# HaploConduct/HaploConduct

Measured on AMD Instinct MI355X. Metric: candidate overlaps scored/sec (edge-calc scoring pass: compute_overlap + overlap_score + admission class, candidates resident in HBM; the whole stage from the overlaps text: stage_end_to_end), higher is better.
Workload: dtype f64

## Files before the change

### haploconduct_amd/_native.py

```python
import ctypes as C
import os

_HERE = os.path.dirname(os.path.abspath(__file__))
lib_path = os.path.join(_HERE, "csrc", "libhcedge.so")


class HcError(RuntimeError):
    def __init__(self, status, where=""):
        self.status = status
        try:
            msg = lib.hc_strerror(status).decode()
            detail = lib.hc_last_error().decode()
        except Exception:
            msg, detail = "?", ""
        super().__init__(f"{where}: {msg} ({status}) {detail}".strip())


if not os.path.exists(lib_path):
    raise ImportError(
        f"{lib_path} is missing: build it with `python -c 'import __graft_entry__ as g; g.build()'` "
        "or `make -C haploconduct_amd/csrc`.  haploconduct_amd has no CPU fallback."
    )

try:
# ... 64 lines not shown
    "hc_block_destroy": (C.c_int, [_vp]),
    "hc_text_set_ids": (C.c_int, [_vp, _vp, C.c_uint32]),
    "hc_textblock_create": (C.c_int, [_vp, C.c_uint64, C.POINTER(_vp)]),
    "hc_textblock_buffer": (_vp, [_vp]),
    "hc_textblock_submit": (C.c_int, [_vp, C.c_uint64, C.c_uint64, C.c_uint64]),
    "hc_textblock_submit_from": (C.c_int, [_vp, _vp, C.c_uint64, _vp, C.c_uint64, _vp, C.c_uint64]),
    "hc_linechain_create": (C.c_int, [_vp, C.c_uint64, C.POINTER(_vp)]),
    "hc_linechain_destroy": (C.c_int, [_vp]),
    "hc_textblock_wait": (C.c_int, [_vp, C.POINTER(hc_text_result)]),
    "hc_textblock_list_nonplain": (C.c_int, [_vp, C.c_uint32]),
    "hc_textblock_destroy": (C.c_int, [_vp]),
    "hc_textblock_regrown": (C.c_uint64, [_vp]),
    "hc_textblock_reserve_rows": (C.c_int, [_vp, C.c_uint64]),
    "hc_graph_begin": (C.c_int, [_vp]),
    "hc_graph_append": (C.c_int, [_vp, _vp, C.c_uint64]),
    "hc_graph_resolve": (C.c_int, [_vp, _vp, C.c_uint64, C.c_uint64, _vp, C.c_uint32, C.POINTER(hc_graph_counts)]),
    "hc_graph_fetch": (C.c_int, [_vp, _vp, _vp, _vp, _vp, _vp, _vp, _vp]),
    "hc_reset": (C.c_int, [_vp, _vp]),
    "hc_set_comm_reserve": (C.c_int, [_vp, C.c_uint32]),
    "hc_comm_gate_device": (C.c_int, [_vp, _vp, C.c_uint32]),
    "hc_compact_pack_device": (C.c_int, [_vp, _vp, C.c_uint64, _vp, _vp, C.c_uint64, C.c_uint64, _vp, _vp]),
    "hc_pack_rows_device": (C.c_int, [_vp, _vp, _vp, _vp, C.c_uint64, C.c_uint64, _vp, _vp]),
    "hc_score_batch_compact": (C.c_int, [_vp, _vp, C.c_uint64, _vp, _vp, C.c_uint64, C.POINTER(C.c_uint64)]),
    "hc_set_reorder": (C.c_int, [_vp, C.c_int]),
    "hc_host_alloc": (C.c_int, [_vp, C.POINTER(_vp), C.c_uint64]),
    "hc_host_free": (C.c_int, [_vp, _vp]),
    "hc_time_score_kernel": (C.c_int, [_vp, C.c_uint32, _vp, C.c_uint64, _vp, C.c_int, C.POINTER(C.c_float)]),
    "hc_count_positions_device": (C.c_int, [_vp, C.c_uint32, _vp, C.c_uint64, C.POINTER(C.c_uint64), C.POINTER(C.c_uint64)]),
    "hc_finalize": (C.c_int, [C.POINTER(hc_settings), _vp, C.POINTER(C.c_double), C.POINTER(C.c_double), C.POINTER(C.c_uint32)]),
    "hc_finalize_batch": (C.c_int, [C.POINTER(hc_settings), _vp, C.c_uint64, _vp, _vp, _vp]),
    "hc_get_info": (C.c_int, [_vp, C.POINTER(C.c_uint32), C.POINTER(C.c_uint64)] + [C.POINTER(C.c_double)] * 4),
    "hc_get_kernel_info": (C.c_int, [_vp, C.c_char_p, C.c_uint32]),
    "hc_get_kernel_info_for": (C.c_int, [_vp, C.c_uint64, C.c_char_p, C.c_uint32]),
    "hc_dev_radix_sort": (C.c_int, [C.c_uint32, C.c_uint32, _vp, _vp, _vp, _vp, C.c_uint64, C.c_int, C.c_int]),
    "hc_dev_exclusive_sum": (C.c_int, [C.c_uint32, _vp, _vp, C.c_uint64]),
    "hc_dev_select_flagged": (C.c_int, [_vp, C.c_uint64, _vp, C.POINTER(C.c_uint64)]),
    "hc_dev_unique_u64": (C.c_int, [_vp, C.c_uint64, _vp, C.POINTER(C.c_uint64)]),
}
for _name, (_res, _args) in _sig.items():
    _f = getattr(lib, _name)
    _f.restype = _res
    _f.argtypes = _args


def check(status, where=""):
    if status != 0:
        raise HcError(status, where)


def device_count():
    return int(lib.hc_device_count())


def version():
    return lib.hc_version().decode()
```

### haploconduct_amd/csrc/hc_api.cpp

```cpp
#include <hip/hip_runtime.h>

#include <chrono>
#include <cmath>
#include <cstdio>
#include <cstdlib>
#include <cstring>
#include <thread>
#include <array>
#include <limits>
#include <new>
#include <string>
#include <vector>

#include "../../include/hcedge.h"
#include "hc_ctx.h"

static thread_local std::string g_last_error;

static int fail(int status, const std::string& what) {
    g_last_error = what;
    return status;
}
namespace hc {
int set_last_error(int status, const std::string& what) { return fail(status, what); }
// ... 35 lines not shown
        case HC_ERR_ARG: return "invalid argument";
        case HC_ERR_NOMEM: return "out of memory";
        case HC_ERR_HIP: return "HIP runtime error";
        case HC_ERR_NO_DEVICE: return "no HIP device (libhcedge has no CPU fallback)";
        case HC_ERR_STATE: return "call order violated";
        case HC_ERR_BAD_READ: return "malformed read set";
        case HC_ERR_BAD_OVERLAP: return "malformed overlap record";
        case HC_ERR_IO: return "I/O error";
        case HC_ERR_FORMAT: return "input format the reference rejects";
        case HC_ERR_DATA: return "overlap touches a base/quality the reference asserts on";
        case HC_ERR_NOT_ON_DEVICE: return "not decided on the device (the host's route takes the input)";
        default: return "unknown status";
    }
}

const char* hc_last_error(void) { return g_last_error.c_str(); }

int hc_device_count(void) {
    int n = 0;
    if (hipGetDeviceCount(&n) != hipSuccess) return 0;
    return n;
}

static void apply_settings(hc_ctx* c, const hc_settings* settings) {
    c->settings = *settings;
    c->params.edge = make_band(settings->edge_threshold);
    c->params.ov = make_band(settings->ov_threshold);
    c->params.merge_contigs = settings->merge_contigs;
    c->params.min_read_len = settings->min_read_len;
    c->params.flags = (settings->edge_threshold < 0 ? kParamEdgeAlways : 0u) | (settings->ov_threshold < 0 ? kParamOvAlways : 0u);
    c->params.rec_fmt = HC_REC_FULL;
    c->params.pad = 0;
    c->params.n_dev = nullptr;
}

static int create_ctx(hc_ctx* c, const hc_settings* settings) {
    c->settings = *settings;
    c->device = settings->device;
    HC_HIP(hipSetDevice(c->device));
    hipDeviceProp_t prop;
    HC_HIP(hipGetDeviceProperties(&prop, c->device));
    c->n_cu = prop.multiProcessorCount > 0 ? (uint32_t)prop.multiProcessorCount : 256u;
    HC_HIP(hipStreamCreateWithFlags(&c->stream, hipStreamNonBlocking));
    HC_HIP(hipEventCreate(&c->ev0));
    HC_HIP(hipEventCreate(&c->ev1));
    HC_HIP(hipMalloc((void**)&c->d_totals, 2 * sizeof(unsigned long long)));
    HC_HIP(hc::set_score_kernel_lds_limit());
    apply_settings(c, settings);
    return HC_OK;
}

int hc_create(hc_ctx** out, const hc_settings* settings) {
    if (!out || !settings) return fail(HC_ERR_ARG, "hc_create: null argument");
    *out = nullptr;
    int n = 0;
    if (hipGetDeviceCount(&n) != hipSuccess || n <= 0)
        return fail(HC_ERR_NO_DEVICE, "hc_create: no HIP device visible");
    if (settings->device < 0 || settings->device >= n) return fail(HC_ERR_ARG, "hc_create: device ordinal out of range");
    hc_ctx* c = new (std::nothrow) hc_ctx();
    if (!c) return fail(HC_ERR_NOMEM, "hc_create: host allocation failed");
    const int rc = create_ctx(c, settings);
    if (rc != HC_OK) {
        const std::string why = g_last_error;
        hc_destroy(c);
        return fail(rc, why);
    }
// ... 2 lines not shown
}

static void free_store(hc_ctx* c, bool scratch_too = true) {
    if (scratch_too) {
        for (auto& sl : c->finder_scratch) {
            if (sl.p) (void)hipFree(sl.p);
            sl.p = nullptr;
            sl.cap = 0;
        }
        for (auto& sl : c->ingest_scratch) {
            if (sl.p) (void)hipFree(sl.p);
            sl.p = nullptr;
            sl.cap = 0;
        }
        if (c->d_found_lines) (void)hipFree(c->d_found_lines);
        c->d_found_lines = nullptr;
        c->found_lines_cap = 0;
        if (c->d_found) (void)hipFree(c->d_found);
        c->d_found = nullptr;
        c->found_cap = 0;
    }
    c->n_found = 0;
    c->found_valid = false;
    if (c->d_sym) (void)hipFree(c->d_sym);
    if (c->d_reads) (void)hipFree(c->d_reads);
    if (c->d_lut) (void)hipFree(c->d_lut);
    if (c->d_inv_n) (void)hipFree(c->d_inv_n);
    c->d_inv_n = nullptr;
    c->d_sym = nullptr;
    c->d_reads = nullptr;
    c->d_lut = nullptr;
    c->have_reads = false;
    c->store_bytes = 0;
}

int hc_destroy(hc_ctx* c) {
    if (!c) return HC_OK;
    (void)hipSetDevice(c->device);
    if (c->stream) (void)hipStreamSynchronize(c->stream);
    free_store(c);
    if (c->d_in) (void)hipFree(c->d_in);
    if (c->d_out) (void)hipFree(c->d_out);
    if (c->d_totals) (void)hipFree(c->d_totals);
    if (c->d_started) (void)hipFree(c->d_started);
    if (c->d_sort) (void)hipFree(c->d_sort);
    if (c->d_sort_tmp) (void)hipFree(c->d_sort_tmp);
    if (c->d_compact_tmp) (void)hipFree(c->d_compact_tmp);
    if (c->d_compact_idx) (void)hipFree(c->d_compact_idx);
    if (c->d_compact_res) (void)hipFree(c->d_compact_res);
    if (c->ev0) (void)hipEventDestroy(c->ev0);
    if (c->ev1) (void)hipEventDestroy(c->ev1);
    if (c->scratch_done) (void)hipEventDestroy(c->scratch_done);
    for (int t = 0; t < 2; t++) {
        if (c->graph.h_stage[t]) (void)hipHostFree(c->graph.h_stage[t]);
        if (c->h_ingest[t]) (void)hipHostFree(c->h_ingest[t]);
        if (c->graph.stage_free[t]) (void)hipEventDestroy(c->graph.stage_free[t]);
    }
    for (void* h : c->h_sfo_text)
        if (h) (void)hipHostFree(h);
    for (hipStream_t s : c->text_copy_stream)
        if (s) (void)hipStreamDestroy(s);
    if (c->stream) (void)hipStreamDestroy(c->stream);
    delete c;
    return HC_OK;
}

// ... 232 lines not shown
        for (uint32_t r = 0; r < n_reads; r++) {
            const uint32_t q = read_first_seq[r];
            if (read_first_seq[r + 1] - q == 2) {
                c->seq_refs[q] = hc::SeqRef{sym_off[q], seq_len[q], n_single + pair_no, rc_delta[q], 0};
                c->seq_refs[q + 1] = hc::SeqRef{sym_off[q + 1], seq_len[q + 1], n_single + n_pairs + pair_no, rc_delta[q + 1], 0};
                pair_no++;
            } else {
                c->seq_refs[q] = hc::SeqRef{sym_off[q], seq_len[q], r, rc_delta[q], 0};
            }
        }
    }
    c->view.sym = c->d_sym;
    c->view.reads = c->d_reads;
    c->view.n_reads = n_reads;
    c->view.n_seq = n_seq;
    c->view.K = K;
    c->view.symbytes = symbytes;
    c->view.lut_bytes = (uint32_t)(lut.size() * sizeof(double));
    c->view.inv_n = c->d_inv_n;
    c->view.inv_len = (uint32_t)inv_n.size();
    c->store_bytes = sym_bytes_total;
    c->view.store_bytes = sym_bytes_total;
    {
        bool same_len = n_seq > 0;
        for (uint32_t q = 1; q < n_seq && same_len; q++) same_len = seq_len[q] == seq_len[0];
        uint32_t n_single = 0;
        for (uint32_t r = 0; r < n_reads; r++) n_single += read_first_seq[r + 1] - read_first_seq[r] == 1;
        c->view.regular = (same_len && c->singles_first && !any_bad_base) ? 1u : 0u;
        if (const char* v = getenv("HC_REGULAR_STORE")) c->view.regular = c->view.regular && atoi(v) != 0;
        c->view.ulen = same_len ? seq_len[0] : 0u;
        c->view.n_single = n_single;
        c->view.seq_syms = same_len ? (uint32_t)(2 * hc::slot_stride(seq_len[0], symbytes, slot_align)) : 0u;
    }
    c->have_reads = true;
    {
        uint32_t lmin = 0, lmax = 0;
        if (n_seq) {
            std::vector<uint32_t> sorted_len(seq_len.begin(), seq_len.begin() + n_seq);
            const size_t k5 = (size_t)n_seq * 5 / 100, k95 = std::min<size_t>(n_seq - 1, (size_t)n_seq * 95 / 100);
            std::nth_element(sorted_len.begin(), sorted_len.begin() + k5, sorted_len.end());
            lmin = sorted_len[k5];
            std::nth_element(sorted_len.begin(), sorted_len.begin() + k95, sorted_len.end());
            lmax = sorted_len[k95];
        }
        c->len_p5 = lmin;
        c->len_p95 = lmax;
        c->view.balance = (n_seq && lmax > 2u * lmin && total / n_seq > 350) ? 1u : 0u;
        if (const char* b = getenv("HC_BALANCE")) c->view.balance = atoi(b) != 0;
    }
    c->coop_fetch = true;
    if (const char* v = getenv("HC_FETCH_GROUP")) {
        c->coop_fetch = !strcmp(v, "coop");
        c->fetch_group = atoi(v) == 2 ? 2 : 4;
    } else {
        const uint64_t mean_len = n_seq ? total / n_seq : 0;
        c->fetch_group = (mean_len > 600 || symbytes == 2) ? 2 : 4;
        const uint32_t lmin = c->len_p5, lmax = c->len_p95;
        uint32_t n_pairs = 0;
        for (uint32_t r = 0; r < n_reads; r++) n_pairs += read_first_seq[r + 1] - read_first_seq[r] == 2;
        const bool short_mixed_singles = n_seq && n_pairs == 0 && lmax > 2u * lmin && mean_len <= 300 && !c->view.balance;
        c->coop_fetch = !short_mixed_singles;
        if (short_mixed_singles) c->fetch_group = 2;
    }
    c->view.long_rows = (n_seq && total / n_seq > 600) ? 1u : 0u;
    return HC_OK;
}

static bool host_batch_is_ordered(const void* in, size_t rec_bytes, uint64_t n) {
    if (n < 2) return true;
    const uint64_t samples = n - 1 < 4096 ? n - 1 : 4096;
    const uint64_t step = (n - 2) / samples > 0 ? (n - 2) / samples : 1;
    uint64_t share = 0;
    for (uint64_t k = 0; k < samples; k++) {
        const uint32_t* a = (const uint32_t*)((const char*)in + k * step * rec_bytes);
        const uint32_t* b = (const uint32_t*)((const char*)in + (k * step + 1) * rec_bytes);
        share += (a[0] == b[0]) | (a[0] == b[1]) | (a[1] == b[0]) | (a[1] == b[1]);
    }
    return share * 2 >= samples;
}

static int ensure_sort_workspace(hc_ctx* c, uint64_t n) {
    if (n <= c->sort_cap) return HC_OK;
    if (c->d_sort) (void)hipFree(c->d_sort);
    if (c->d_sort_tmp) (void)hipFree(c->d_sort_tmp);
    c->d_sort = nullptr;
    c->d_sort_tmp = nullptr;
    c->sort_cap = 0;
    c->sort_tmp_bytes = hc::reorder_temp_bytes((uint32_t)n);
    HC_HIP(hipMalloc((void**)&c->d_sort, 4 * n * sizeof(uint32_t)));
    HC_HIP(hipMalloc(&c->d_sort_tmp, c->sort_tmp_bytes ? c->sort_tmp_bytes : 16));
    c->sort_cap = n;
    return HC_OK;
}

}

int hc_ctx_score(hc_ctx* c, uint32_t fmt, const void* d_in, uint64_t n, void* d_out, hipStream_t s, bool reorder,
                 hc_gather_row* rows, unsigned long long* row_count, uint64_t cap, uint64_t base_index, const unsigned long long* n_dev,
                 const hc_line_rec* lines_in, hc_line_rec* lines_out, hc_bucket_ws* bucket) {
    const bool want_perm = reorder && n > 1 && n < (1ull << 31);
    const bool want_bucket = c->view.balance && c->coop_fetch && n < (1ull << 32);
    const bool want_segments = rows && !lines_in && c->coop_fetch;
    const bool ctx_scratch = want_perm || (want_bucket && !bucket) || want_segments;
    if (ctx_scratch) {
        if (!c->scratch_done) HC_HIP(hipEventCreateWithFlags(&c->scratch_done, hipEventDisableTiming));
        if (c->scratch_used && c->scratch_stream != s) HC_HIP(hipStreamWaitEvent(s, c->scratch_done, 0));
    }
    const uint32_t* perm = nullptr;
    if (want_perm) {
        int rc = ensure_sort_workspace(c, n);
        if (rc) return rc;
        uint32_t* keys_in = c->d_sort;
        uint32_t* keys_out = c->d_sort + c->sort_cap;
        uint32_t* idx_in = c->d_sort + 2 * c->sort_cap;
        uint32_t* perm_out = c->d_sort + 3 * c->sort_cap;
        HC_HIP(hc::launch_reorder(c->view.n_reads, fmt, d_in, (uint32_t)n, keys_in, keys_out, idx_in, perm_out, c->d_sort_tmp,
                                  c->sort_tmp_bytes, s));
        perm = perm_out;
    }
    hc::ScoreParams prm = c->params;
    prm.rec_fmt = fmt;
    prm.pad = 0;
    prm.n_dev = n_dev;
    uint32_t *bperm = nullptr, *bqueue = nullptr;
    if (want_bucket) {
        hc_bucket_ws* ws = bucket ? bucket : &c->bucket;
        int rc = ws->ensure(n);
        if (rc) return rc;
        bperm = ws->perm();
        bqueue = ws->queue();
    }
    hc_gather_row* seg_buf = nullptr;
    uint32_t* seg_count = nullptr;
    uint64_t seg_total = 0;
    if (want_segments) {
        seg_total = 2 * cap + hc::kSinkMaxGroups * 512;
        if (seg_total * sizeof(hc_gather_row) > c->sink_rows.cap && c->scratch_used) HC_HIP(hipEventSynchronize(c->scratch_done));
        int rc = c->sink_rows.ensure(seg_total * sizeof(hc_gather_row));
        if (rc) return rc;
        if (!c->sink_counts.p) {
            if ((rc = c->sink_counts.ensure((hc::kSinkMaxGroups + 2) * sizeof(uint32_t))) != HC_OK) return rc;
            HC_HIP(hipMemsetAsync(c->sink_counts.p, 0, (hc::kSinkMaxGroups + 2) * sizeof(uint32_t), s));
        }
        seg_buf = c->sink_rows.as<hc_gather_row>();
        seg_count = c->sink_counts.as<uint32_t>();
    }
    if (want_segments && c->sink_dirty) {
        HC_HIP(hipMemsetAsync(c->sink_counts.as<uint32_t>() + hc::kSinkMaxGroups, 0, 2 * sizeof(uint32_t), s));
        c->sink_dirty = false;
    }
    const uint32_t cus = c->comm_reserve && c->comm_reserve < c->n_cu ? c->n_cu - c->comm_reserve : c->n_cu;
    unsigned long long* started = (rows && !lines_in) ? c->d_started : nullptr;
    uint32_t started_groups = 0;
    const hipError_t le = hc::launch_score(c->view, prm, c->d_lut, d_in, n, (hc_result_rec*)d_out, perm, cus, c->coop_fetch ? 0 : c->fetch_group, c->fetch_group, rows,
                                           row_count, cap, base_index, s, lines_in, lines_out, bperm, bqueue, seg_buf, seg_count, seg_total, &c->sink_turn, started,
                                           &started_groups);
    if (le != hipSuccess) {
        if (want_segments) c->sink_dirty = true;
        return hc::set_last_error(HC_ERR_HIP, std::string("launch_score: ") + hipGetErrorString(le));
    }
    if (started) c->started_target += started_groups;
    if (ctx_scratch) {
        HC_HIP(hipEventRecord(c->scratch_done, s));
        c->scratch_stream = s;
        c->scratch_used = true;
    }
    return HC_OK;
}

extern "C" {

int hc_set_reorder(hc_ctx* c, int mode) {
    if (!c || mode < HC_REORDER_NEVER || mode > HC_REORDER_AUTO) return fail(HC_ERR_ARG, "hc_set_reorder: bad argument");
    c->reorder_mode = mode;
    return HC_OK;
}

int hc_score_batch_device(hc_ctx* c, const void* d_in, uint64_t n, void* d_out, void* hip_stream) {
    if (!c) return fail(HC_ERR_ARG, "hc_score_batch_device: null context");
    if (!c->have_reads) return fail(HC_ERR_STATE, "hc_score_batch_device: hc_set_reads has not been called");
    if (n == 0) return HC_OK;
    if (!d_in || !d_out) return fail(HC_ERR_ARG, "hc_score_batch_device: null buffer");
    HC_HIP(hipSetDevice(c->device));
    hipStream_t s = hip_stream ? (hipStream_t)hip_stream : c->stream;
    return hc_ctx_score(c, HC_REC_FULL, d_in, n, d_out, s, c->reorder_mode == HC_REORDER_ALWAYS, nullptr, nullptr, 0, 0);
}

int hc_score_cands_device(hc_ctx* c, const void* d_in, uint64_t n, void* d_out, void* hip_stream) {
    if (!c) return fail(HC_ERR_ARG, "hc_score_cands_device: null context");
    if (!c->have_reads) return fail(HC_ERR_STATE, "hc_score_cands_device: hc_set_reads has not been called");
    if (n == 0) return HC_OK;
    if (!d_in || !d_out) return fail(HC_ERR_ARG, "hc_score_cands_device: null buffer");
    HC_HIP(hipSetDevice(c->device));
    hipStream_t s = hip_stream ? (hipStream_t)hip_stream : c->stream;
    return hc_ctx_score(c, HC_REC_COMPACT, d_in, n, d_out, s, c->reorder_mode == HC_REORDER_ALWAYS, nullptr, nullptr, 0, 0);
}

void hc_pack_cands(const hc_overlap_rec* in, uint64_t n, hc_cand_rec* out) {
    for (uint64_t i = 0; i < n; i++) {
        const hc_overlap_rec& r = in[i];
        const uint32_t p1 = r.pos1 < HC_CAND_POS_MASK ? r.pos1 : HC_CAND_POS_MASK;
        const uint32_t p2 = r.pos2 < HC_CAND_POS_MASK ? r.pos2 : HC_CAND_POS_MASK;
        const uint32_t oc = r.ord == '-' ? 0u : (r.ord == '1' ? 1u : (r.ord == '2' ? 2u : 3u));
        out[i].read1 = r.read1;
        out[i].read2 = r.read2;
        out[i].pos1_bits = p1 | (r.ori1 ? 1u << 28 : 0u) | (r.ori2 ? 1u << 29 : 0u) | (oc << 30);
        out[i].pos2_bits = p2;
// ... 329 lines not shown
```

### haploconduct_amd/csrc/hc_ctx.h

```cpp
#pragma once
#include <hip/hip_runtime.h>

#include <atomic>
#include <string>
#include <vector>

#include "../../include/hcedge.h"
#include "hc_device.h"
#include "hc_overlap_finder.h"

namespace hc {
hipError_t launch_encode(uint32_t symbytes, const uint8_t* bases, const uint8_t* quals, const uint64_t* raw_off,
                         const uint64_t* seq_off, const uint32_t* rc_delta, const uint8_t* qmap, uint32_t n_seq, uint32_t K, void* sym,
                         uint8_t* seq_bad, const uint32_t* read_first_seq, uint32_t n_reads, ReadDesc* descs, uint32_t slot_align,
                         hipStream_t stream);
hipError_t launch_score(const StoreView& st, const ScoreParams& prm, const double* lut_g, const void* in, uint64_t n,
                        hc_result_rec* out, const uint32_t* perm, uint32_t n_cu, int fetch_group, int lane_fetch_group, hc_gather_row* rows,
                        unsigned long long* row_count, uint64_t cap, uint64_t base_index, hipStream_t stream,
                        const hc_line_rec* lines_in = nullptr, hc_line_rec* lines_out = nullptr, uint32_t* bucket_perm = nullptr,
                        uint32_t* bucket_queue = nullptr, hc_gather_row* seg_buf = nullptr, uint32_t* seg_count = nullptr, uint64_t seg_total_rows = 0,
                        uint32_t* spill_turn = nullptr, unsigned long long* started = nullptr, uint32_t* started_groups = nullptr);
hipError_t set_score_kernel_lds_limit();
std::string describe_score_kernel(const StoreView& st, int fetch_group, int lane_fetch_group, uint32_t n_cu = 256, uint64_t n = 0);
size_t compact_temp_bytes(uint32_t n);
hipError_t launch_compact(const hc_result_rec* res, uint32_t n, uint32_t* idx_out, unsigned long long* count_out, void* temp,
                          size_t temp_bytes, hipStream_t stream);
hipError_t launch_narrow_payload(const void* in32, uint64_t cap, void* out24, uint32_t n_cu, hipStream_t stream);
hipError_t launch_pack_rows(const hc_result_rec* res, const uint32_t* idx, const unsigned long long* count, uint64_t cap, uint64_t base,
                            hc_gather_row* rows, uint32_t n_cu, hipStream_t stream);
hipError_t launch_pack_header(const unsigned long long* count, hc_gather_row* header, hipStream_t stream);
hipError_t launch_gather_results(const hc_result_rec* res, const uint32_t* idx, const unsigned long long* count,
                                 hc_result_rec* out, uint32_t n_cu, hipStream_t stream);
size_t reorder_temp_bytes(uint32_t n);
hipError_t launch_reorder(uint32_t n_reads, uint32_t fmt, const void* in, uint32_t n, uint32_t* keys_in, uint32_t* keys_out,
                          uint32_t* idx_in, uint32_t* perm_out, void* temp, size_t temp_bytes, hipStream_t stream);
hipError_t launch_count_positions(const StoreView& st, uint32_t min_read_len, uint32_t fmt, const void* in, uint64_t n,
                                  unsigned long long* totals, hipStream_t stream);
hipError_t launch_kept_rows(const hc_result_rec* res, uint64_t n, const unsigned long long* n_dev, uint64_t base_index, uint32_t* tile_cnt,
                            uint32_t* tile_off, hc_gather_row* rows, uint64_t cap, unsigned long long* count, const hc_line_rec* lines_in,
                            hc_line_rec* lines_out, hipStream_t stream, const uint32_t* text_tally = nullptr,
                            unsigned long long* text_counters = nullptr);
hipError_t launch_flush_text_rows(const void* rows, void* rows_mapped, const void* lines, void* lines_mapped, const unsigned long long* count,
                                  uint64_t cap, const unsigned long long* counters, unsigned long long* counters_mapped, uint32_t n_cu,
                                  hipStream_t stream);
hipError_t launch_comm_gate(const unsigned long long* started, unsigned long long target, uint32_t timeout_us, hipStream_t stream);
hipError_t launch_flush_rows(const void* src, void* dst_mapped, const unsigned long long* count, uint64_t cap, uint32_t row_bytes, uint32_t n_cu,
                             hipStream_t stream);

int set_last_error(int status, const std::string& what);
}

#define HC_HIP(call)                                                                                   \
    do {                                                                                               \
        hipError_t e__ = (call);                                                                       \
        if (e__ != hipSuccess)                                                                         \
            return hc::set_last_error(HC_ERR_HIP, std::string(#call) + ": " + hipGetErrorString(e__)); \
    } while (0)

struct hc_scratch {
    void* p = nullptr;
    size_t cap = 0;
    bool host = false;
    int ensure(size_t bytes) {
        if (bytes <= cap) return HC_OK;
        release();
        const size_t want = bytes + bytes / 8;
        if (host) HC_HIP(hipHostMalloc(&p, want, hipHostMallocMapped));
        else HC_HIP(hipMalloc(&p, want));
        cap = want;
        return HC_OK;
    }
    void release() {
        if (p) (void)(host ? hipHostFree(p) : hipFree(p));
        p = nullptr;
        cap = 0;
    }
    template <typename T>
    T* as() const { return (T*)p; }
    hc_scratch() = default;
    hc_scratch(const hc_scratch&) = delete;
// ... 24 lines not shown
    double* d_lut = nullptr;
    double* d_inv_n = nullptr;
    uint32_t len_p5 = 0, len_p95 = 0;
    uint64_t store_bytes = 0;
    hc::StoreView view{};
    hc::ScoreParams params{};
    std::vector<hc::SeqRef> seq_refs;
    bool singles_first = true;
    struct Scratch {
        void* p = nullptr;
        size_t cap = 0;
    } finder_scratch[24], ingest_scratch[12];
    void* h_ingest[2] = {nullptr, nullptr};
    size_t h_ingest_cap = 0;
    void* h_sfo_text[3] = {nullptr, nullptr, nullptr};
    hc_sfo_rec* d_found = nullptr;
    uint64_t found_cap = 0;
    uint64_t n_found = 0;
    hc_line_rec* d_found_lines = nullptr;
    uint64_t found_lines_cap = 0;
    double found_err = -1;
    uint32_t found_min = 0, found_flags = 0;
    bool found_valid = false;
    void* d_in = nullptr;
    void* d_out = nullptr;
    uint64_t ws_cap = 0;
    unsigned long long* d_totals = nullptr;
    int reorder_mode = HC_REORDER_AUTO;
    uint32_t* d_sort = nullptr;
    void* d_sort_tmp = nullptr;
    size_t sort_tmp_bytes = 0;
    uint64_t sort_cap = 0;
    hc_bucket_ws bucket;
    hc_scratch sink_rows, sink_counts;
    uint32_t sink_turn = 0;
    bool sink_dirty = false;
    uint32_t comm_reserve = 0;
    unsigned long long* d_started = nullptr;
    unsigned long long started_target = 0;

    hipEvent_t scratch_done = nullptr;
    hipStream_t scratch_stream = nullptr;
    bool scratch_used = false;
    void* d_compact_tmp = nullptr;
    size_t compact_tmp_bytes = 0;
    uint32_t* d_compact_idx = nullptr;
    hc_result_rec* d_compact_res = nullptr;
    uint64_t compact_cap = 0;
    hc_scratch id_table, id_keys;
    uint64_t id_size = 0;
    int id_shift = 0, id_direct = 1;
    bool have_ids = false;
    struct Graph {
        hc_scratch adm, E, key0, key1, idx0, idx1, keep, incl, tied, counters, surv, k32a, k32b, k64a, k64b, tmp_idx, o_out, o_in,
            out_off, in_off, edges_out, in_nodes, vtx, temp, tied_list;
        uint64_t n_vertices = 0, n_edges = 0, n_tied = 0;
        uint64_t n_appended = 0;
        bool valid = false;
        void* h_stage[2] = {nullptr, nullptr};
        size_t stage_cap[2] = {0, 0};
        hipEvent_t stage_free[2] = {nullptr, nullptr};
        int stage_turn = 0;
    } graph;
};

int hc_ctx_score(hc_ctx* c, uint32_t fmt, const void* d_in, uint64_t n, void* d_out, hipStream_t s, bool reorder,
// ... 6 lines not shown
```

### haploconduct_amd/csrc/hc_device.h

```cpp
#pragma once
#include <stdint.h>

namespace hc {

constexpr uint64_t kSinkMaxGroups = 4096;
constexpr uint32_t kCodeN = 4;
constexpr uint32_t kCodeBadQual = 6;
constexpr uint32_t kCodeBadBase = 7;

constexpr uint32_t kReadPaired = 1u;
constexpr uint32_t kReadBadBase1 = 2u;
constexpr uint32_t kReadBadBase2 = 4u;

__host__ __device__ inline uint64_t slot_stride(uint32_t len, uint32_t symbytes, uint32_t align) {
    uint64_t bytes = (uint64_t)len * symbytes;
    bytes = ((bytes + 15) & ~(uint64_t)15) + 32;
    bytes = (bytes + align - 1) & ~(uint64_t)(align - 1);
    return bytes / symbytes;
}

struct ReadDesc {
    uint64_t off1, off2;
    uint32_t len1, len2;
    uint32_t flags;
// ... 26 lines not shown
                                               17, 59, 46, 42, 58, 43, 30, 41, 38, 19, 61, 56, 29, 53, 31, 47, 23, 49, 18, 60, 51, 52, 57, 22};
constexpr uint8_t kWide7RankLabel[kWide7MaxK] = {8,  15, 4,  19, 24, 35, 49, 31, 6,  42, 20, 9,  61, 37, 18, 58, 16, 22, 23, 21,
                                                 45, 33, 54, 14, 25, 5,  47, 12, 57, 7,  43, 38, 63, 34, 28, 50, 27, 51, 44, 10,
                                                 26, 29, 11, 32, 60, 40, 39, 56, 13, 46, 36, 55, 17, 62, 53, 59, 52, 48, 41, 30};
__host__ __device__ inline uint32_t lut_lg(uint32_t K) {
    return K + 2 <= 8 ? 3u : (K + 2 <= 16 ? 4u : (K + 2 <= 32 ? 5u : (K <= kWideMaxK ? 6u : (K <= kWide7MaxK ? 7u : 6u))));
}
__host__ __device__ inline uint32_t wide_first(uint32_t lg) { return lg == 7 ? kWide7First : kWideFirst; }
__host__ __device__ inline uint32_t sym_bytes_for(uint32_t K) { return K <= kWide7MaxK ? 1u : 2u; }
__host__ __device__ inline uint32_t lut_tri(uint32_t Kp) { return Kp * (Kp + 1u) / 2u; }
__host__ __device__ inline uint32_t lut_addr_u16(uint32_t Kp, uint32_t qa, uint32_t qb, uint32_t m) {
    const uint32_t hi = qa > qb ? qa : qb, lo = qa > qb ? qb : qa;
    return (m * lut_tri(Kp) + hi * (hi + 1u) / 2u + lo) * 8u;
}
__host__ __device__ inline uint32_t lut_doubles_u8(uint32_t lg) { return lg == 3 ? 2048u : (lg >= 6 ? 8192u : (2u << (2 * lg))); }
__host__ __device__ inline uint32_t lut_addr_u8(uint32_t lg, uint32_t qa, uint32_t qb, uint32_t m) {
    if (lg == 3) return (qa << 11) | (m << 10) | ((qa & 3u) << 6) | (((qb ^ qa) & 7u) << 3);
    if (lg >= 6) return (m << 15) | (qa << 9) | ((((qb ^ qa) >> 5) & 1u) << 8) | ((((qb ^ qa) ^ (qa >> 1)) & 31u) << 3);
    return m * (8u << (2 * lg)) + qa * (8u << lg) + ((qb ^ qa) & ((1u << lg) - 1u)) * 8u;
}

struct Band {
    double lo, hi;
};

struct ScoreParams {
    Band edge, ov;
    double merge_contigs;
    uint32_t min_read_len;
    uint32_t flags;
    uint32_t rec_fmt;
    uint32_t pad;
    const unsigned long long* n_dev;
};

}
```

### haploconduct_amd/csrc/hc_kernels.hip

```cpp
#include <hip/hip_runtime.h>
#include <stdint.h>
#include <stdlib.h>

#include <algorithm>
#include <type_traits>
#include <cstdio>
#include <string>

#include "../../include/hcedge.h"
#include "hc_device.h"
#include "hc_resolve.h"

#ifndef HC_COOP_AUX_A
#define HC_COOP_AUX_A 0
#endif
#ifndef HC_COOP_AUX_B
#define HC_COOP_AUX_B 0
#endif

#ifndef HC_ABLATE
#define HC_ABLATE 0
#endif

namespace hc {
// ... 1060 lines not shown
    }
    extern __shared__ __attribute__((aligned(16))) double lut_s[];
    if ((uint32_t)(uintptr_t)(__attribute__((address_space(3))) void*)lut_s != 0u) __builtin_trap();
    const uint32_t lut_n = st.lut_bytes >> 3;
    load_log_table<SymT, LG>(lut_s, lut_g, lut_n, threadIdx.x, WG);
    constexpr bool kScratchInTable = sizeof(SymT) == 1 && LG >= 6 && WG == (int)kWideDmaLanes;
    uint32_t* scratch = kScratchInTable ? (uint32_t*)((char*)lut_s + kWideDmaScratch) : (uint32_t*)(lut_s + lut_n);
    if (kScratchInTable) __syncthreads();
    const uint32_t seg_counter = (uint32_t)(uintptr_t)(__attribute__((address_space(3))) void*)(scratch + 24);
    if (threadIdx.x == 0) {
        scratch[24] = 0;
        scratch[29] = 0;
        if (DYN && !WQ) scratch[26] = atomicAdd(queue, 1u);
        if (sink.started) atomicAdd(sink.started, 1ull);
    }
    __syncthreads();
    const uint32_t stage_base = coop_stage_base(st.lut_bytes, WG);
    const uint32_t stage = (uint32_t)__builtin_amdgcn_readfirstlane(
        (int)(stage_base + (threadIdx.x >> 6) * (DEPTH == 0 ? 2u * kStageBytesPerWave : kStageBytesPerWave)));
    const SymT* sym = (const SymT*)st.sym;
    const uint32_t Kp = st.K + 2u;
    const uint32_t fmt = prm.rec_fmt;
    const __amdgpu_buffer_rsrc_t rsrc = __builtin_amdgcn_make_buffer_rsrc((void*)st.sym, 0, (uint32_t)st.store_bytes, 0x00020000);
    const uint32_t oob = (uint32_t)st.store_bytes;
    const uint32_t tid = threadIdx.x;
    const uint64_t stride = (uint64_t)gridDim.x * WG;
    const uint32_t n_tiles = DYN ? (uint32_t)((n_hint + kBucketTile - 1) / kBucketTile) : 0u;
    const uint32_t n_pieces = n_tiles * (kBucketTile / WG);
    uint32_t q_ahead = 0, iter = 0;
    const uint32_t wq_steps = WQ ? ((prm.pad >> 8) & 0xFu) : 0u;
    const uint32_t dq_pieces = (DYN && WQ && blockIdx.x < n_pieces) ? (n_pieces - blockIdx.x + gridDim.x - 1) / gridDim.x : 0u;
    const uint32_t wq_items = !WQ ? 0u : (DYN ? dq_pieces * (uint32_t)(WG / 64) : (uint32_t)((n + 64ull * wq_steps - 1) / (64ull * wq_steps)));
    const uint32_t wq_per = !WQ ? 0u : (DYN ? wq_items : (wq_items + gridDim.x - 1) / gridDim.x);
    const uint32_t wq_first = DYN ? 0u : blockIdx.x * wq_per, wq_end = wq_first + wq_per < wq_items ? wq_first + wq_per : wq_items;
    uint32_t wq_item = 0, wq_next_raw = 0, wq_k = 0;
    auto wq_pull = [&]() -> uint32_t {
        uint32_t t = 0;
        if ((tid & 63u) == 0) t = lds_add_rtn(seg_counter + 20u, 1u);
        return t;
    };
    if (WQ) {
        wq_item = wq_first + (tid >> 6);
        if (wq_item < wq_end) wq_next_raw = wq_pull();
    }
    for (uint64_t block_base = (uint64_t)blockIdx.x * WG;; block_base += stride, ++iter) {
        uint64_t slot;
        if (WQ) {
            if (wq_k == wq_steps) {
                wq_item = wq_first + (uint32_t)(WG / 64) + (uint32_t)__builtin_amdgcn_readfirstlane((int)wq_next_raw);
                wq_k = 0;
                if (wq_item < wq_end) wq_next_raw = wq_pull();
            }
            if (wq_item >= wq_end) break;
            if (DYN) {
                const uint32_t k = wq_item / (uint32_t)(WG / 64), w = wq_item - k * (uint32_t)(WG / 64);
                const uint32_t q = blockIdx.x + k * gridDim.x;
                const uint32_t piece = q / n_tiles, tile = q - piece * n_tiles;
                slot = (uint64_t)tile * kBucketTile + piece * WG + w * 64u + (tid & 63u);
            } else {
                slot = ((uint64_t)wq_item * wq_steps + wq_k) * 64u + (tid & 63u);
            }
            ++wq_k;
        } else if (DYN) {
            const uint32_t q = scratch[26 + (iter & 1u)];
            if (q >= n_pieces) break;
            if (tid == 0) q_ahead = atomicAdd(queue, 1u);
            const uint32_t piece = q / n_tiles, tile = q - piece * n_tiles;
            slot = (uint64_t)tile * kBucketTile + piece * WG + tid;
        } else {
            if (block_base >= n) break;
            slot = block_base + tid;
        }
        uint64_t i = 0;
        int ns = -2;
        uint32_t a0 = 0, b0 = 0, l0 = 0, a1 = 0, b1 = 0, l1 = 0;
        if (slot < n) {
            i = perm ? (uint64_t)perm[slot] : slot;
            const Cand rec = load_cand(in, i, fmt);
            if (st.regular) {
                ns = resolve_regular32<(int)sizeof(SymT)>(st, prm.min_read_len, rec, a0, b0, l0, a1, b1, l1);
            } else {
                Sub sub0{}, sub1{};
                ns = resolve<(int)sizeof(SymT)>(st, rec, sub0, sub1);
                if (ns >= 1) {
                    a0 = (uint32_t)((sub0.offA + sub0.pos) * sizeof(SymT));
                    b0 = (uint32_t)(sub0.offB * sizeof(SymT));
                    l0 = sub_positions(sub0, prm.min_read_len) | (sub0.fatal << 31);
                }
                if (ns == 2) {
                    a1 = (uint32_t)((sub1.offA + sub1.pos) * sizeof(SymT));
                    b1 = (uint32_t)(sub1.offB * sizeof(SymT));
                    l1 = sub_positions(sub1, prm.min_read_len) | (sub1.fatal << 31);
                }
// ... 517 lines not shown
```

### haploconduct_amd/scorer.py

```python
import ctypes as C

import numpy as np

from . import _native as N
from .records import ADMIT_DTYPE, CAND_DTYPE, OVERLAP_DTYPE, REC_COMPACT, REC_FULL, RESULT_DTYPE, ROW_DTYPE, TEXT_REJECT_DTYPE, TEXT_ROW_DTYPE, Settings


def _ptr(a):
    return C.c_void_p(a.ctypes.data)


class EdgeScorer:
    def __init__(self, settings: Settings = None):
        self.settings = settings or Settings()
        self._cs = self.settings.to_c()
        self._ctx = C.c_void_p()
        N.check(N.lib.hc_create(C.byref(self._ctx), C.byref(self._cs)), "hc_create")
        self._reads = None

    def close(self):
        if getattr(self, "_ctx", None) is not None and self._ctx.value:
            N.lib.hc_destroy(self._ctx)
            self._ctx = C.c_void_p()

    def __del__(self):
        try:
            self.close()
        except Exception:
            pass

    def __enter__(self):
        return self

    def __exit__(self, *a):
        self.close()

    def set_reads(self, reads):
        self._reads = reads
        N.check(
            N.lib.hc_set_reads(self._ctx, _ptr(reads.bases), _ptr(reads.quals), _ptr(reads.seq_off),
                               _ptr(reads.read_first_seq), reads.n_reads),
            "hc_set_reads",
        )

    def info(self):
        k, sb = C.c_uint32(), C.c_uint64()
        d = [C.c_double() for _ in range(4)]
        N.check(N.lib.hc_get_info(self._ctx, C.byref(k), C.byref(sb), *[C.byref(x) for x in d]), "hc_get_info")
        return {"qual_alphabet": k.value, "store_bytes": sb.value, "x_edge": (d[0].value, d[1].value),
                "x_ov": (d[2].value, d[3].value)}

    def kernel_info(self, n=0):
        buf = C.create_string_buffer(768)
        N.check(N.lib.hc_get_kernel_info_for(self._ctx, int(n), buf, 768), "hc_get_kernel_info_for")
        return buf.value.decode()

    def set_reorder(self, mode):
        N.check(N.lib.hc_set_reorder(self._ctx, int(mode)), "hc_set_reorder")

    def score_batch(self, overlaps):
        ov = np.ascontiguousarray(overlaps, dtype=OVERLAP_DTYPE)
        out = np.empty(ov.shape[0], dtype=RESULT_DTYPE)
        N.check(N.lib.hc_score_batch(self._ctx, _ptr(ov), ov.shape[0], _ptr(out)), "hc_score_batch")
        return out

    @staticmethod
    def pack_cands(overlaps):
        ov = np.ascontiguousarray(overlaps, dtype=OVERLAP_DTYPE)
        out = np.empty(ov.shape[0], dtype=CAND_DTYPE)
        N.lib.hc_pack_cands(_ptr(ov), ov.shape[0], _ptr(out))
        return out

    def score_cands(self, cands):
        cd = np.ascontiguousarray(cands, dtype=CAND_DTYPE)
        out = np.empty(cd.shape[0], dtype=RESULT_DTYPE)
        N.check(N.lib.hc_score_cands(self._ctx, _ptr(cd), cd.shape[0], _ptr(out)), "hc_score_cands")
        return out

    def score_cands_device(self, d_in_ptr, n, d_out_ptr, stream=None):
        N.check(N.lib.hc_score_cands_device(self._ctx, C.c_void_p(d_in_ptr), n, C.c_void_p(d_out_ptr), C.c_void_p(stream or 0)),
                "hc_score_cands_device")

    def score_blocks(self, cands, block=250000, in_flight=2):
        cd = np.ascontiguousarray(cands, dtype=CAND_DTYPE)
        n = cd.shape[0]
        blocks = []
        for _ in range(in_flight):
            b = C.c_void_p()
# ... 242 lines not shown
```

### include/hcedge.h

```cpp
#ifndef HCEDGE_H_
#define HCEDGE_H_

#include <stddef.h>
#include <stdint.h>

#ifdef __cplusplus
extern "C" {
#endif

typedef enum hc_status {
    HC_OK = 0,
    HC_ERR_ARG = -1,
    HC_ERR_NOMEM = -2,
    HC_ERR_HIP = -3,
    HC_ERR_NO_DEVICE = -4,
    HC_ERR_STATE = -5,
    HC_ERR_BAD_READ = -6,
    HC_ERR_BAD_OVERLAP = -7,
    HC_ERR_IO = -8,
    HC_ERR_FORMAT = -9,
    HC_ERR_DATA = -10,
    HC_ERR_NOT_ON_DEVICE = -11
} hc_status;

// ... 112 lines not shown
    uint32_t OLA, OLB, K;
    uint32_t inverted;
} hc_sfo_rec;
int hc_find_overlaps(hc_ctx* ctx, double err_rate, uint32_t min_overlap, uint32_t flags, hc_sfo_rec* out, uint64_t cap,
                     uint64_t* n_out);
int hc_found_to_overlaps(hc_ctx* ctx, const char* out_path, uint64_t num_singles, uint64_t num_pairs, uint64_t* n_lines);
int hc_set_found_records(hc_ctx* ctx, const hc_sfo_rec* recs, uint64_t n);
int hc_set_found_from_sfo_text(hc_ctx* ctx, const char* text, uint64_t n_bytes, uint64_t* n_records);
struct hc_line_rec;
int hc_found_lines_fetch(hc_ctx* ctx, const struct hc_line_rec* d_lines, uint64_t n, struct hc_line_rec* out);
int hc_found_to_lines_device(hc_ctx* ctx, uint64_t num_singles, uint64_t num_pairs, const struct hc_line_rec** d_lines, uint64_t* n_lines);

int hc_compact_pack_device(hc_ctx* ctx, const void* d_results, uint64_t n, void* d_indices, void* d_count, uint64_t cap,
                           uint64_t base_index, void* d_payload, void* hip_stream);

int hc_score_pack_device(hc_ctx* ctx, uint32_t rec_fmt, const void* d_in, uint64_t n, void* d_out, uint64_t cap, uint64_t base_index,
                         void* d_payload, void* hip_stream);

int hc_narrow_payload_device(hc_ctx* ctx, const void* d_payload, uint64_t cap, void* d_payload24, void* hip_stream);

int hc_set_comm_reserve(hc_ctx* ctx, uint32_t cus);
int hc_comm_gate_device(hc_ctx* ctx, void* hip_stream, uint32_t timeout_us);

int hc_score_batch_compact(hc_ctx* ctx, const hc_overlap_rec* in, uint64_t n, uint32_t* idx_out, hc_result_rec* res_out,
                           uint64_t cap, uint64_t* n_out);

int hc_time_score_kernel(hc_ctx* ctx, uint32_t rec_fmt, const void* d_in, uint64_t n, void* d_out, int iters, float* ms_per_launch);

int hc_count_positions_device(hc_ctx* ctx, uint32_t rec_fmt, const void* d_in, uint64_t n, uint64_t* total_positions,
                              uint64_t* total_subs);

int hc_get_kernel_info(hc_ctx* ctx, char* buf, uint32_t cap);
int hc_get_kernel_info_for(hc_ctx* ctx, uint64_t n, char* buf, uint32_t cap);

int hc_dev_radix_sort(uint32_t key_bytes, uint32_t val_bytes, const void* keys, const void* vals, void* keys_out, void* vals_out, uint64_t n,
                      int begin_bit, int end_bit);
int hc_dev_exclusive_sum(uint32_t elem_bytes, const void* in, void* out, uint64_t n);
int hc_dev_select_flagged(const uint8_t* flags, uint64_t n, uint32_t* idx_out, uint64_t* count);
int hc_dev_unique_u64(const uint64_t* in, uint64_t n, uint64_t* out, uint64_t* count);

int hc_finalize(const hc_settings* s, const hc_result_rec* r, double* score, double* mismatch_rate, uint32_t* cls);

int hc_finalize_batch(const hc_settings* s, const hc_result_rec* r, uint64_t n, double* score, double* mismatch_rate,
                      uint32_t* cls);

typedef struct hc_line_rec {
    uint64_t id1, id2;
    uint32_t pos1, pos2, perc1, perc2, len1, len2;
    uint8_t ord, ori1, ori2, type1, type2, pad[3];
} hc_line_rec;
typedef struct hc_text_row {
    hc_gather_row row;
    hc_line_rec line;
} hc_text_row;
typedef struct hc_text_reject {
    uint32_t line_index, pad;
    hc_line_rec line;
} hc_text_reject;
typedef struct hc_text_nonplain {
    uint32_t line_index;
    uint32_t begin;
    uint32_t length;
    uint32_t pad;
} hc_text_nonplain;
typedef struct hc_text_result {
    uint64_t n_lines;
// ... 75 lines not shown
```

Before: 15.51 billion.

## Reorder candidate scoring by minimizer-based read locality and XCD-grouped work

At read upload, each read gets a minimizer hash key (min over 16-mers) and reads are sorted by it to form a locality order. For large compact-format candidate batches sorted by hot read, the scorer builds a permutation that visits candidate groups in that read order, so reads with shared sequence content are scored close in time. Work items are also interleaved across blocks in groups of 8, which looks intended to match MI355X XCD block placement and improve per-XCD L2 reuse. This adds several small index kernels per call and a per-batch scratch buffer, and it falls back to identity order if the input is not sorted.

```diff
diff --git a/haploconduct_amd/_native.py b/haploconduct_amd/_native.py
--- a/haploconduct_amd/_native.py
+++ b/haploconduct_amd/_native.py
@@ -120,6 +120,7 @@
     "hc_get_info": (C.c_int, [_vp, C.POINTER(C.c_uint32), C.POINTER(C.c_uint64)] + [C.POINTER(C.c_double)] * 4),
     "hc_get_kernel_info": (C.c_int, [_vp, C.c_char_p, C.c_uint32]),
     "hc_get_kernel_info_for": (C.c_int, [_vp, C.c_uint64, C.c_char_p, C.c_uint32]),
+    "hc_get_locality_order": (C.c_int, [_vp, _vp, C.c_uint64, C.POINTER(C.c_uint64)]),
     "hc_dev_radix_sort": (C.c_int, [C.c_uint32, C.c_uint32, _vp, _vp, _vp, _vp, C.c_uint64, C.c_int, C.c_int]),
     "hc_dev_exclusive_sum": (C.c_int, [C.c_uint32, _vp, _vp, C.c_uint64]),
     "hc_dev_select_flagged": (C.c_int, [_vp, C.c_uint64, _vp, C.POINTER(C.c_uint64)]),
diff --git a/haploconduct_amd/csrc/hc_api.cpp b/haploconduct_amd/csrc/hc_api.cpp
--- a/haploconduct_amd/csrc/hc_api.cpp
+++ b/haploconduct_amd/csrc/hc_api.cpp
@@ -91,6 +91,7 @@
     c->params.rec_fmt = HC_REC_FULL;
     c->params.pad = 0;
     c->params.n_dev = nullptr;
+    c->params.order_off = nullptr;
 }
 
 static int create_ctx(hc_ctx* c, const hc_settings* settings) {
@@ -159,6 +160,7 @@
     c->d_lut = nullptr;
     c->have_reads = false;
     c->store_bytes = 0;
+    c->loc_reads = 0;
 }
 
 int hc_destroy(hc_ctx* c) {
@@ -457,6 +459,20 @@
         c->view.n_single = n_single;
         c->view.seq_syms = same_len ? (uint32_t)(2 * hc::slot_stride(seq_len[0], symbytes, slot_align)) : 0u;
     }
+    c->loc_reads = 0;
+    if (c->view.regular && n_reads > 1) {
+        const size_t tmp = hc::locality_order_temp_bytes(n_reads);
+        const size_t keys_bytes = 2 * sizeof(uint64_t) * (size_t)n_reads, idx_bytes = sizeof(uint32_t) * (((size_t)n_reads + 3) & ~(size_t)3);
+        int rc = c->loc_tmp.ensure(keys_bytes + idx_bytes + tmp);
+        if (rc == HC_OK) rc = c->loc_order.ensure(sizeof(uint32_t) * (size_t)n_reads);
+        if (rc) return rc;
+        uint64_t* keys = c->loc_tmp.as<uint64_t>();
+        uint32_t* idx = (uint32_t*)(keys + 2 * (size_t)n_reads);
+        HC_HIP(hc::launch_locality_order(d_bases, d_raw_off, d_first, n_reads, keys, keys + n_reads, idx, c->loc_order.as<uint32_t>(),
+                                         (char*)idx + idx_bytes, tmp, c->stream));
+        HC_HIP(hipStreamSynchronize(c->stream));
+        c->loc_reads = n_reads;
+    }
     c->have_reads = true;
     {
         uint32_t lmin = 0, lmax = 0;
@@ -520,13 +536,23 @@
 
 }
 
+static constexpr uint64_t kLocalityMinCandidates = 8000000;
+static bool locality_wanted(uint64_t n) {
+    const char* e = getenv("HC_LOCALITY");
+    if (e && atoi(e) == 0) return false;
+    const char* m = getenv("HC_LOCALITY_MIN");
+    return n >= (m ? strtoull(m, nullptr, 10) : kLocalityMinCandidates);
+}
+
 int hc_ctx_score(hc_ctx* c, uint32_t fmt, const void* d_in, uint64_t n, void* d_out, hipStream_t s, bool reorder,
                  hc_gather_row* rows, unsigned long long* row_count, uint64_t cap, uint64_t base_index, const unsigned long long* n_dev,
                  const hc_line_rec* lines_in, hc_line_rec* lines_out, hc_bucket_ws* bucket) {
     const bool want_perm = reorder && n > 1 && n < (1ull << 31);
     const bool want_bucket = c->view.balance && c->coop_fetch && n < (1ull << 32);
     const bool want_segments = rows && !lines_in && c->coop_fetch;
-    const bool ctx_scratch = want_perm || (want_bucket && !bucket) || want_segments;
+    const bool want_loc = !want_perm && !want_bucket && !rows && !lines_in && !bucket && fmt == HC_REC_COMPACT && c->coop_fetch && c->view.regular &&
+                          c->loc_reads == c->view.n_reads && c->loc_reads > 1 && n > 1 && n < (1ull << 32) && locality_wanted(n);
+    const bool ctx_scratch = want_perm || (want_bucket && !bucket) || want_segments || want_loc;
     if (ctx_scratch) {
         if (!c->scratch_done) HC_HIP(hipEventCreateWithFlags(&c->scratch_done, hipEventDisableTiming));
         if (c->scratch_used && c->scratch_stream != s) HC_HIP(hipStreamWaitEvent(s, c->scratch_done, 0));
@@ -543,10 +569,28 @@
                                   c->sort_tmp_bytes, s));
         perm = perm_out;
     }
+    const uint32_t* order_off = nullptr;
+    if (want_loc) {
+        const uint32_t R = c->loc_reads;
+        const size_t head = ((size_t)R + 2 + (size_t)R + 1 + 1 + 3) & ~(size_t)3;
+        const size_t tmp = hc::locality_index_temp_bytes(R);
+        if ((head + n) * sizeof(uint32_t) > c->loc_ws.cap && c->scratch_used) HC_HIP(hipEventSynchronize(c->scratch_done));
+        int rc = c->loc_ws.ensure((head + n) * sizeof(uint32_t));
+        if (rc == HC_OK) rc = c->loc_tmp.ensure(tmp ? tmp : 16);
+        if (rc) return rc;
+        uint32_t* flag = c->loc_ws.as<uint32_t>();
+        uint32_t* bounds = flag + 1;
+        uint32_t* starts = bounds + R + 2;
+        uint32_t* lperm = c->loc_ws.as<uint32_t>() + head;
+        HC_HIP(hc::launch_locality_index(c->loc_order.as<uint32_t>(), R, d_in, n, n_dev, bounds, starts, flag, lperm, c->loc_tmp.p, tmp, s));
+        perm = lperm;
+        order_off = flag;
+    }
     hc::ScoreParams prm = c->params;
     prm.rec_fmt = fmt;
     prm.pad = 0;
     prm.n_dev = n_dev;
+    prm.order_off = order_off;
     uint32_t *bperm = nullptr, *bqueue = nullptr;
     if (want_bucket) {
         hc_bucket_ws* ws = bucket ? bucket : &c->bucket;
@@ -598,6 +642,17 @@
 int hc_set_reorder(hc_ctx* c, int mode) {
     if (!c || mode < HC_REORDER_NEVER || mode > HC_REORDER_AUTO) return fail(HC_ERR_ARG, "hc_set_reorder: bad argument");
     c->reorder_mode = mode;
+    return HC_OK;
+}
+
+int hc_get_locality_order(hc_ctx* c, uint32_t* out, uint64_t cap, uint64_t* n) {
+    if (!c || !n || (cap && !out)) return fail(HC_ERR_ARG, "hc_get_locality_order: bad argument");
+    *n = c->have_reads ? c->loc_reads : 0;
+    const uint64_t k = std::min<uint64_t>(cap, *n);
+    if (k) {
+        HC_HIP(hipSetDevice(c->device));
+        HC_HIP(hipMemcpy(out, c->loc_order.p, k * sizeof(uint32_t), hipMemcpyDeviceToHost));
+    }
     return HC_OK;
 }
 
diff --git a/haploconduct_amd/csrc/hc_ctx.h b/haploconduct_amd/csrc/hc_ctx.h
--- a/haploconduct_amd/csrc/hc_ctx.h
+++ b/haploconduct_amd/csrc/hc_ctx.h
@@ -46,6 +46,13 @@
 hipError_t launch_comm_gate(const unsigned long long* started, unsigned long long target, uint32_t timeout_us, hipStream_t stream);
 hipError_t launch_flush_rows(const void* src, void* dst_mapped, const unsigned long long* count, uint64_t cap, uint32_t row_bytes, uint32_t n_cu,
                              hipStream_t stream);
+
+size_t locality_order_temp_bytes(uint32_t n_reads);
+hipError_t launch_locality_order(const uint8_t* bases, const uint64_t* raw_off, const uint32_t* read_first_seq, uint32_t n_reads, uint64_t* keys_a,
+                                 uint64_t* keys_b, uint32_t* idx, uint32_t* order_out, void* temp, size_t temp_bytes, hipStream_t stream);
+size_t locality_index_temp_bytes(uint32_t n_reads);
+hipError_t launch_locality_index(const uint32_t* order, uint32_t n_reads, const void* in, uint64_t n, const unsigned long long* n_dev, uint32_t* bounds,
+                                 uint32_t* start, uint32_t* flag, uint32_t* perm, void* temp, size_t temp_bytes, hipStream_t stream);
 
 int set_last_error(int status, const std::string& what);
 }
@@ -136,6 +143,8 @@
     size_t sort_tmp_bytes = 0;
     uint64_t sort_cap = 0;
     hc_bucket_ws bucket;
+    hc_scratch loc_order, loc_ws, loc_tmp;
+    uint32_t loc_reads = 0;
     hc_scratch sink_rows, sink_counts;
     uint32_t sink_turn = 0;
     bool sink_dirty = false;
diff --git a/haploconduct_amd/csrc/hc_device.h b/haploconduct_amd/csrc/hc_device.h
--- a/haploconduct_amd/csrc/hc_device.h
+++ b/haploconduct_amd/csrc/hc_device.h
@@ -82,6 +82,7 @@
     uint32_t rec_fmt;
     uint32_t pad;
     const unsigned long long* n_dev;
+    const uint32_t* order_off;
 };
 
 }
diff --git a/haploconduct_amd/csrc/hc_kernels.hip b/haploconduct_amd/csrc/hc_kernels.hip
--- a/haploconduct_amd/csrc/hc_kernels.hip
+++ b/haploconduct_amd/csrc/hc_kernels.hip
@@ -1116,7 +1116,22 @@
     const uint32_t dq_pieces = (DYN && WQ && blockIdx.x < n_pieces) ? (n_pieces - blockIdx.x + gridDim.x - 1) / gridDim.x : 0u;
     const uint32_t wq_items = !WQ ? 0u : (DYN ? dq_pieces * (uint32_t)(WG / 64) : (uint32_t)((n + 64ull * wq_steps - 1) / (64ull * wq_steps)));
     const uint32_t wq_per = !WQ ? 0u : (DYN ? wq_items : (wq_items + gridDim.x - 1) / gridDim.x);
-    const uint32_t wq_first = DYN ? 0u : blockIdx.x * wq_per, wq_end = wq_first + wq_per < wq_items ? wq_first + wq_per : wq_items;
+    uint32_t wq_first = DYN ? 0u : blockIdx.x * wq_per, wq_end = wq_first + wq_per < wq_items ? wq_first + wq_per : wq_items;
+    uint32_t xq_base = 0, xq_stride = 0;
+    if (WQ && !DYN && prm.order_off) {
+        if (*prm.order_off) {
+            perm = nullptr;
+        } else if (wq_items) {
+            const uint32_t G = gridDim.x, g = blockIdx.x & 7u, l = blockIdx.x >> 3, q = G >> 3, r = G & 7u;
+            const uint32_t m = q + (g < r ? 1u : 0u);
+            const uint32_t g_start = (g * q + (g < r ? g : r)) * wq_per;
+            const uint32_t g_end = g_start + m * wq_per < wq_items ? g_start + m * wq_per : wq_items;
+            wq_first = 0;
+            wq_end = g_end > g_start + l ? (g_end - g_start - l + m - 1) / m : 0u;
+            xq_base = g_start + l;
+            xq_stride = m;
+        }
+    }
     uint32_t wq_item = 0, wq_next_raw = 0, wq_k = 0;
     auto wq_pull = [&]() -> uint32_t {
         uint32_t t = 0;
@@ -1142,7 +1157,8 @@
                 const uint32_t piece = q / n_tiles, tile = q - piece * n_tiles;
                 slot = (uint64_t)tile * kBucketTile + piece * WG + w * 64u + (tid & 63u);
             } else {
-                slot = ((uint64_t)wq_item * wq_steps + wq_k) * 64u + (tid & 63u);
+                const uint32_t item = xq_stride ? xq_base + xq_stride * wq_item : wq_item;
+                slot = ((uint64_t)item * wq_steps + wq_k) * 64u + (tid & 63u);
             }
             ++wq_k;
         } else if (DYN) {
diff --git a/haploconduct_amd/csrc/hc_locality.hip b/haploconduct_amd/csrc/hc_locality.hip
--- /dev/null
+++ b/haploconduct_amd/csrc/hc_locality.hip
@@ -0,0 +1,128 @@
+#include <hip/hip_runtime.h>
+#include <stdint.h>
+
+#include "../../include/hcedge.h"
+#include "hc_prims.h"
+
+namespace hc {
+
+namespace {
+
+constexpr uint32_t kLocK = 16;
+constexpr uint64_t kLocHashMul = 0x9E3779B97F4A7C15ull;
+constexpr int kLocKeyBits = 44;
+constexpr uint64_t kLocNoKey = (1ull << kLocKeyBits) - 1;
+constexpr uint32_t kLocSamples = 1u << 16;
+
+__device__ __forceinline__ uint32_t base_code(uint8_t b) {
+    return b == 'C' ? 1u : (b == 'G' ? 2u : (b == 'T' ? 3u : 0u));
+}
+
+__global__ __launch_bounds__(256) void locality_key_kernel(const uint8_t* __restrict__ bases, const uint64_t* __restrict__ raw_off,
+                                                           const uint32_t* __restrict__ read_first_seq, uint32_t n_reads,
+                                                           uint64_t* __restrict__ keys, uint32_t* __restrict__ idx) {
+    const uint32_t r = blockIdx.x * blockDim.x + threadIdx.x;
+    if (r >= n_reads) return;
+    const uint32_t q = read_first_seq[r];
+    const uint64_t off = raw_off[q], len = raw_off[q + 1] - off;
+    uint64_t best = kLocNoKey;
+    uint32_t kmer = 0;
+    for (uint64_t j = 0; j < len; j++) {
+        kmer = (kmer << 2) | base_code(bases[off + j]);
+        if (j + 1 >= kLocK) {
+            const uint64_t h = ((uint64_t)kmer * kLocHashMul) >> (64 - kLocKeyBits);
+            best = h < best ? h : best;
+        }
+    }
+    keys[r] = best;
+    idx[r] = r;
+}
+
+__device__ __forceinline__ uint32_t hot_read(const void* in, uint64_t i, uint32_t n_reads) {
+    const uint2 p = *((const uint2*)((const hc_cand_rec*)in + i));
+    const uint32_t h = p.x < p.y ? p.x : p.y;
+    return h < n_reads ? h : n_reads;
+}
+
+__global__ __launch_bounds__(256) void locality_bounds_kernel(const void* __restrict__ in, uint64_t n, const unsigned long long* __restrict__ n_dev,
+                                                              uint32_t n_reads, uint32_t* __restrict__ bounds, uint32_t* __restrict__ flag) {
+    const uint64_t ne = n_dev ? (*n_dev < n ? *n_dev : n) : n;
+    const uint32_t t = blockIdx.x * blockDim.x + threadIdx.x;
+    if (t <= n_reads + 1u) {
+        uint64_t b;
+        if (t == 0) b = 0;
+        else if (t == n_reads + 1u) b = ne;
+        else {
+            uint64_t lo = 0, hi = ne;
+            while (lo < hi) {
+                const uint64_t mid = (lo + hi) >> 1;
+                if (hot_read(in, mid, n_reads) < t) lo = mid + 1;
+                else hi = mid;
+            }
+            b = lo;
+        }
+        bounds[t] = (uint32_t)b;
+    }
+    if (t < kLocSamples && ne >= 2) {
+        const uint64_t i = (ne - 1) * t / kLocSamples;
+        if (hot_read(in, i, n_reads) > hot_read(in, i + 1, n_reads)) atomicOr(flag, 1u);
+    }
+}
+
+__global__ __launch_bounds__(256) void locality_lengths_kernel(const uint32_t* __restrict__ order, uint32_t n_reads, const uint32_t* __restrict__ bounds,
+                                                               uint32_t* __restrict__ len, uint32_t* __restrict__ flag) {
+    const uint32_t k = blockIdx.x * blockDim.x + threadIdx.x;
+    if (k > n_reads) return;
+    const uint32_t h = k < n_reads ? order[k] : n_reads;
+    const uint32_t lo = bounds[h], hi = bounds[h + 1];
+    if (hi < lo) atomicOr(flag, 1u);
+    len[k] = hi >= lo ? hi - lo : 0u;
+}
+
+__global__ __launch_bounds__(256) void locality_fill_kernel(const uint32_t* __restrict__ order, uint32_t n_reads, const uint32_t* __restrict__ bounds,
+                                                            const uint32_t* __restrict__ start, const uint32_t* __restrict__ flag, uint64_t n,
+                                                            const unsigned long long* __restrict__ n_dev, uint32_t* __restrict__ perm) {
+    const uint64_t ne = n_dev ? (*n_dev < n ? *n_dev : n) : n;
+    if (*flag) {
+        const uint64_t stride = (uint64_t)gridDim.x * blockDim.x;
+        for (uint64_t i = (uint64_t)blockIdx.x * blockDim.x + threadIdx.x; i < ne; i += stride) perm[i] = (uint32_t)i;
+        return;
+    }
+    const uint32_t k = (uint32_t)(((uint64_t)blockIdx.x * blockDim.x + threadIdx.x) >> 6), lane = threadIdx.x & 63u;
+    if (k > n_reads) return;
+    const uint32_t h = k < n_reads ? order[k] : n_reads;
+    const uint32_t lo = bounds[h], len = bounds[h + 1] - lo, s = start[k];
+    for (uint32_t j = lane; j < len; j += 64u)
+        if ((uint64_t)s + j < ne) perm[s + j] = lo + j;
+}
+
+}
+
+size_t locality_order_temp_bytes(uint32_t n_reads) { return prims::sort_temp_bytes(n_reads, sizeof(uint64_t), sizeof(uint32_t)); }
+
+hipError_t launch_locality_order(const uint8_t* bases, const uint64_t* raw_off, const uint32_t* read_first_seq, uint32_t n_reads, uint64_t* keys_a,
+                                 uint64_t* keys_b, uint32_t* idx, uint32_t* order_out, void* temp, size_t temp_bytes, hipStream_t stream) {
+    if (n_reads == 0) return hipSuccess;
+    hipLaunchKernelGGL(locality_key_kernel, dim3((n_reads + 255) / 256), dim3(256), 0, stream, bases, raw_off, read_first_seq, n_reads, keys_a, idx);
+    return prims::sort_pairs(temp, temp_bytes, keys_a, keys_b, idx, order_out, n_reads, 0, kLocKeyBits, stream);
+}
+
+size_t locality_index_temp_bytes(uint32_t n_reads) { return prims::scan_temp_bytes((uint64_t)n_reads + 1, sizeof(uint32_t)); }
+
+hipError_t launch_locality_index(const uint32_t* order, uint32_t n_reads, const void* in, uint64_t n, const unsigned long long* n_dev, uint32_t* bounds,
+                                 uint32_t* start, uint32_t* flag, uint32_t* perm, void* temp, size_t temp_bytes, hipStream_t stream) {
+    hipError_t e = hipMemsetAsync(flag, 0, sizeof(uint32_t), stream);
+    if (e != hipSuccess) return e;
+    const uint32_t threads = n_reads + 2u > kLocSamples ? n_reads + 2u : kLocSamples;
+    hipLaunchKernelGGL(locality_bounds_kernel, dim3((threads + 255) / 256), dim3(256), 0, stream, in, n, n_dev, n_reads, bounds, flag);
+    hipLaunchKernelGGL(locality_lengths_kernel, dim3((n_reads + 1u + 255) / 256), dim3(256), 0, stream, (const uint32_t*)order, n_reads,
+                       (const uint32_t*)bounds, start, flag);
+    e = prims::exclusive_sum(temp, temp_bytes, start, start, (uint64_t)n_reads + 1, stream);
+    if (e != hipSuccess) return e;
+    const uint64_t fill_threads = ((uint64_t)n_reads + 1) * 64;
+    hipLaunchKernelGGL(locality_fill_kernel, dim3((uint32_t)((fill_threads + 255) / 256)), dim3(256), 0, stream, order, n_reads, (const uint32_t*)bounds,
+                       (const uint32_t*)start, (const uint32_t*)flag, n, n_dev, perm);
+    return hipGetLastError();
+}
+
+}
diff --git a/haploconduct_amd/scorer.py b/haploconduct_amd/scorer.py
--- a/haploconduct_amd/scorer.py
+++ b/haploconduct_amd/scorer.py
@@ -54,6 +54,13 @@
         buf = C.create_string_buffer(768)
         N.check(N.lib.hc_get_kernel_info_for(self._ctx, int(n), buf, 768), "hc_get_kernel_info_for")
         return buf.value.decode()
+
+    def locality_order(self):
+        n = C.c_uint64()
+        N.check(N.lib.hc_get_locality_order(self._ctx, None, 0, C.byref(n)), "hc_get_locality_order")
+        out = np.empty(n.value, np.uint32)
+        N.check(N.lib.hc_get_locality_order(self._ctx, out.ctypes.data_as(C.c_void_p), out.size, C.byref(n)), "hc_get_locality_order")
+        return out
 
     def set_reorder(self, mode):
         N.check(N.lib.hc_set_reorder(self._ctx, int(mode)), "hc_set_reorder")
diff --git a/include/hcedge.h b/include/hcedge.h
--- a/include/hcedge.h
+++ b/include/hcedge.h
@@ -168,6 +168,7 @@
 
 int hc_get_kernel_info(hc_ctx* ctx, char* buf, uint32_t cap);
 int hc_get_kernel_info_for(hc_ctx* ctx, uint64_t n, char* buf, uint32_t cap);
+int hc_get_locality_order(hc_ctx* ctx, uint32_t* out, uint64_t cap, uint64_t* n);
 
 int hc_dev_radix_sort(uint32_t key_bytes, uint32_t val_bytes, const void* keys, const void* vals, void* keys_out, void* vals_out, uint64_t n,
                       int begin_bit, int end_bit);
```

Result: faster. 16.92 billion (median of 6 runs) (+9.1%).
